# 5l1v3r1/PBS

Hardware: AMD Instinct MI355X
Metric: co-run slowdown (%) vs solo + aggregate throughput, 4-tenant mix at 1/2/4/8 GPU (higher is better)
Workload: dtype bf16

## Files before the change

csrc/hip/runtime.cpp:

```cpp
#include <hip/hip_runtime.h>
#include <hsa/hsa.h>
#include <hsa/hsa_ext_amd.h>
#include <rocprofiler-sdk-roctx/roctx.h>
#include <x86intrin.h>

#include <algorithm>
#include <atomic>
#include <cmath>
#include <cstdio>
#include <cstdlib>
#include <chrono>
#include <condition_variable>
#include <cstring>
#include <deque>
#include <memory>
#include <mutex>
#include <thread>
#include <vector>

#include "../include/gpbs/gpbs.h"
#include "common.hpp"
#include "hwc_attr.h"

using namespace gpbs_hip;

extern "C" {
int gpbs_adapt_update(gpbs_adapt_state_t*, const gpbs_adapt_params_t*, uint64_t, uint64_t, uint64_t, uint64_t);
int gpbs_hip_gemm_units(int, int);
int gpbs_hip_gemm_fp8_units(int, int);
int gpbs_hwc_sample(uint64_t* out, int nxcd);
int gpbs_hwc_sample_se(uint64_t* se_out, uint64_t* x_out);
int gpbs_hwc_slot_per_se(int k);
int gpbs_hwc_active(void);
int gpbs_hip_gemm_bf16(const void*, const void*, void*, int, int, int, void*, const void*, unsigned, unsigned, void*,
                       void*, int, hipStream_t);
int gpbs_hip_gemm_fp8(const void*, const float*, const void*, const float*, void*, int, int, int, int, void*, const void*,
                      unsigned, unsigned, void*, void*, int, hipStream_t);
int gpbs_hip_stream_copy(const void*, void*, unsigned long long, unsigned, void*, const void*, unsigned, unsigned,
                         void*, void*, int, hipStream_t);
int gpbs_hip_reduce_bf16(const void*, const void*, void*, unsigned long long, unsigned, void*, const void*, unsigned,
                         unsigned, void*, void*, int, hipStream_t);
int gpbs_hip_gemv_bf16(const void*, const void*, void*, int, int, void*, const void*, unsigned, unsigned, void*, void*,
                       int, hipStream_t);
int gpbs_hip_partition_switch(void*, unsigned, const unsigned*, hipStream_t);
int gpbs_hip_counter_reduce(void*, void*, const int*, int, void*, hipStream_t);
int gpbs_hip_adapt(void*, const void*, const void*, const void*, int, const gpbs_adapt_params_t*, int*, hipStream_t);
int gpbs_hip_switch_probe(const void*, int, unsigned*, int, unsigned, unsigned long long, hipStream_t);
int gpbs_hip_hwc_attribute(const void*, void*, void*, void*, hipStream_t);
int gpbs_hip_hwc_attribute2(const void*, void*, void*, void*, hipStream_t, int);
int gpbs_hip_allreduce(const void*, unsigned, unsigned long long, unsigned, void*, const void*, unsigned, unsigned,
                       void*, void*, int, unsigned long long, unsigned long long, hipStream_t);
int gpbs_hip_gang_desc_size(void);
int gpbs_hip_gang_exchange(const void*, unsigned, const void*, void*, void*, unsigned long long, hipStream_t);
int gpbs_hip_coll_desc_size(void);
}

namespace {

// ... 110 lines not shown
    return nullptr;
  }
  volatile u32* w = (volatile u32*)p;
  for (int i = 0; i < 1024; ++i) w[i] = 0;
  _mm_sfence();
  return (PartTable*)p;
}

void bar_write(PartTable* b, const u32* owners, u32 epoch);

void bar_sync(PartTable* b, const PartTable* h) {
  *(volatile u32*)&b->flags = __atomic_load_n(&h->flags, __ATOMIC_ACQUIRE);
  *(volatile u32*)&b->hold = __atomic_load_n(&h->hold, __ATOMIC_ACQUIRE);
  bar_write(b, h->owner, __atomic_load_n(&h->epoch, __ATOMIC_ACQUIRE));
}

void bar_write(PartTable* b, const u32* owners, u32 epoch) {
  volatile u32* o = (volatile u32*)b->owner;
  for (int x = 0; x < kXcds * kCtx; ++x) o[x] = owners[x];
  _mm_sfence();
  *(volatile u32*)&b->epoch = epoch;
  _mm_sfence();
}

struct GpuCtx;
void set_hold(GpuCtx* c, u32 v);

struct GpuCtx {
  int device = 0;
  int part_base = 0;
  int table_mode = 0;
  int spatial = 0;
  PartTable* h_table = nullptr;
  PartTable* d_table = nullptr;
  PartTable* b_table = nullptr;
  u64* d_cnt = nullptr;
  bool cnt_bar = false;
  std::atomic<int> cnt_rows{1};
  u64* d_prev = nullptr;
  u64* h_out = nullptr;
  int* h_ids = nullptr;
  gpbs_adapt_state_t* h_states = nullptr;
  u64* h_spin = nullptr;
  int* h_dirs = nullptr;
  u64* h_adelta = nullptr;
  hipStream_t sched_stream = nullptr;
  gpbs_engine_t* engine = nullptr;
  int nctx = 1;
  int waveprio = 0;
  int lat_half = -1;
  int hold_enable = 0;
  std::mutex hold_mu;
  int holds = 0;
  uint64_t hold_gen = 0;
  std::atomic<uint64_t> hold_raises{0};
  std::atomic<int> cls_cache[kMaxTenants];
  u32 pending[kXcds * kCtx];
  u32 epoch = 0;
  bool red_pending = false;
  int red_n = 0;
  int red_buf = 0;
  int* h_ids2 = nullptr;
  u64* h_out2 = nullptr;
  hipEvent_t red_ev = nullptr;
  int hwc = 0;
  int slot_se[kNumPmc] = {1, 1, 1, 0};
  u64* h_blk = nullptr;
  std::vector<u64> snap_blk, blk_prev;
  std::vector<u64> red_prev;
  std::vector<u64> snap_se;
  std::vector<u64> snap_x;
  std::vector<int64_t> snap_own;
  uint64_t snap_seq = 0, used_seq = 0;
  bool hw_primed = false;
// ... 1228 lines not shown
  std::condition_variable cv, idle_cv;
  int64_t pending = 0;
  int64_t inflight = 0;
  bool stop = false;
  std::deque<int64_t> submit_times;
  gpbs_runner_stats_t st{};
  std::vector<int64_t> lats;
  hipEvent_t ev[16];
  int err = 0;
  uint64_t q_hold[16] = {};

  void hold_drop(int qi) {
    if (q_hold[qi]) {
      hold_release(ctx, q_hold[qi] - 1);
      q_hold[qi] = 0;
    }
  }

  std::atomic<int> phase{0};
  uint8_t q_alt[16] = {};
  int cur_alt = 0;
  u32 q_seq[16] = {};
  u32 coll_seq = 0;
  int64_t q_t0[16] = {};

  struct Work {
    int kind, M, N, K, chunk;
    unsigned long long bytes;
    void *a, *b, *c;
  };
  static int coll_timeout_ms(const Work& w) { return w.K > 0 ? w.K : 5000; }
  Work work(int alt) const {
    if (alt && cfg.alt_kind)
      return Work{cfg.alt_kind, cfg.alt_M, cfg.alt_N, cfg.alt_K, cfg.alt_chunk_bytes, cfg.alt_bytes,
                  cfg.alt_a, cfg.alt_b, cfg.alt_c};
    return Work{cfg.kind, cfg.M, cfg.N, cfg.K, cfg.chunk_bytes, cfg.bytes, cfg.a, cfg.b, cfg.c};
  }

  static u32 unit_total(const Work& w) {
    switch (w.kind) {
      case K_ALLREDUCE: {
        const u64 n8 = w.bytes / 16, chunk8 = (u64)w.chunk / 16, per = (n8 + w.M - 1) / w.M;
        const u64 lo = (u64)w.N * per, hi = std::min(lo + per, n8);
        return hi > lo ? (u32)((hi - lo + chunk8 - 1) / chunk8) : 0u;
      }
      case K_GEMM: return (u32)gpbs_hip_gemm_units(w.M, w.N);
      case K_GEMM_FP8: return (u32)gpbs_hip_gemm_fp8_units(w.M, w.N);
      case K_STREAM:
      case K_REDUCE: return (u32)((w.bytes + w.chunk - 1) / w.chunk);
      case K_GEMV: return (u32)((w.M + 15) / 16);
    }
    return 0;
  }

  hipStream_t pick_se_stream() {
    u32 any = 0, bits = 0;
    for (int x = 0; x < kXcds; ++x)
      for (int e = 0; e < kCtx; ++e)
        if ((__atomic_load_n(&ctx->h_table->owner[kCtx * x + e], __ATOMIC_ACQUIRE) & kOwnerMask) == (u32)cfg.tenant) {
          any |= 1u << e;
          bits |= 1u << (kCtx * x + e);
        }
    const int half = (any & ~0x3u) == 0 ? 0 : ((any & ~0xCu) == 0 ? 1 : -1);
    if (!any || half < 0) return stream;
    if (!key_stream || bits != key_bits || half != key_half) {
      uint32_t m[8];
      se_half_mask(half, m);
      if (key_stream) {
        retire_stream(key_stream);
        masked_pool().release(key_stream, key_load);
      }
      const int64_t tnow = mono_ns();
      key_load = rate_t0 && tnow > rate_t0 ? (double)(st.launches - rate_l0) * 1e9 / (double)(tnow - rate_t0) : 0.0;
      rate_t0 = tnow;
      rate_l0 = st.launches;
      key_stream = masked_acquire_key(m, bits, key_load);
// ... 52 lines not shown
    if (!half_stream[k]) half_stream[k] = make_half_stream(k);
    return half_stream[k] ? half_stream[k] : stream;
  }

  int launch(int qi, hipStream_t stream) {
    WorkQueue* q = d_q + qi;
    const Work w = work(q_alt[qi]);
    const int tm = __atomic_load_n(&ctx->table_mode, __ATOMIC_ACQUIRE);
    const bool dev = tm != 0;
    const void* tab = tm == 1 ? (const void*)ctx->d_table : tm == 2 ? (const void*)ctx->b_table : (const void*)ctx->h_table;
    const bool gate = cfg.gate && !ctx->share.load(std::memory_order_acquire);
    const bool hold = gate && ctx->hold_enable && tm != 1 && w.kind != K_GEMV && ctx->engine &&
                      ctx->cls_cache[cfg.tenant].load(std::memory_order_relaxed) == 1;
    const unsigned mode = (gate ? (cfg.gate == 2 ? GATE_PARK : GATE_TABLE) : GATE_NONE) | (dev ? GATE_DEVTABLE : 0) |
                          (gate && ctx->spatial ? GATE_SPATIAL : 0) |
                          (gate && __atomic_load_n(&ctx->se_mode, __ATOMIC_ACQUIRE) ? GATE_SE : 0) |
                          (cfg.priority > 0 && ctx->waveprio ? GATE_WAVEPRIO : 0) | (hold ? GATE_HOLD : 0);
    const unsigned me = (unsigned)cfg.tenant;
    __atomic_store_n(&h_status[qi], 0u, __ATOMIC_RELEASE);
    st.launches++;
    const int grid = cfg.grid ? cfg.grid : cur_grid;
    switch (w.kind) {
      case K_GEMM:
        return gpbs_hip_gemm_bf16(w.a, w.b, w.c, w.M, w.N, w.K, q, tab, mode, me, ctx->d_cnt, &h_status[qi], grid,
                                  stream);
      case K_GEMM_FP8: {
        const char *aq = (const char*)w.a, *bq = (const char*)w.b;
        return gpbs_hip_gemm_fp8(aq, (const float*)(aq + (size_t)w.M * w.K), bq, (const float*)(bq + (size_t)w.N * w.K),
                                 w.c, w.M, w.N, w.K, 0, q, tab, mode, me, ctx->d_cnt, &h_status[qi], grid, stream);
      }
      case K_STREAM:
        return gpbs_hip_stream_copy(w.a, w.c, w.bytes, (unsigned)w.chunk, q, tab, mode, me, ctx->d_cnt,
                                    &h_status[qi], grid, stream);
      case K_REDUCE:
        return gpbs_hip_reduce_bf16(w.a, w.b, w.c, w.bytes, (unsigned)w.chunk, q, tab, mode, me, ctx->d_cnt,
                                    &h_status[qi], grid, stream);
      case K_GEMV:
        return gpbs_hip_gemv_bf16(w.a, w.b, w.c, w.M, w.K, q, tab, mode, me, ctx->d_cnt, &h_status[qi], grid,
                                  stream);
      case K_ALLREDUCE:
        return gpbs_hip_allreduce(w.a, q_seq[qi], w.bytes, (unsigned)w.chunk, q, tab, mode, me, ctx->d_cnt,
                                  &h_status[qi], grid, (unsigned long long)coll_timeout_ms(w) * 100000ull,
                                  100000ull, stream);
    }
    return -22;
  }

  bool owns_any() {
    if (!cfg.gate || shared()) return true;
    for (int x = 0; x < kXcds * kCtx; ++x)
      if ((__atomic_load_n(&ctx->h_table->owner[x], __ATOMIC_ACQUIRE) & kOwnerMask) == (u32)cfg.tenant) return true;
    return false;
  }

  int wo_qi = -1;
  int64_t q_l0[16] = {};
  int64_t drain_seen_rv = 0;
  int64_t ramp_from = 0;
  static void ewma(std::atomic<int64_t>& a, std::atomic<uint64_t>& n, int64_t v) {
    const int64_t o = a.load(std::memory_order_relaxed);
    a.store(n.load(std::memory_order_relaxed) ? o + (v - o) / 8 : v, std::memory_order_relaxed);
    n.fetch_add(1, std::memory_order_relaxed);
  }
  void note_drain(int qi, int64_t now) {
    if (cfg.tenant < 0 || cfg.tenant >= kMaxTenants) return;
    const int64_t rv = ctx->revoke_ns[cfg.tenant].load(std::memory_order_relaxed);
    if (!rv || rv == drain_seen_rv || rv < q_l0[qi] || now < rv) return;
    const u32 s = __atomic_load_n(&h_status[qi], __ATOMIC_ACQUIRE);
    if ((s & 0x80000000u) && (s & 0x3fffffffu) >= unit_total(work(q_alt[qi]))) return;
    drain_seen_rv = rv;
    const int64_t dr = now - rv;
    if (dr >= 1000000000) return;
    st.drain_sum_ns += dr;
    st.drain_count++;
    if (dr > st.drain_max_ns) st.drain_max_ns = dr;
    ewma(ctx->swc_drain_ns[cfg.tenant], ctx->swc_drain_n[cfg.tenant], dr);
  }
  void note_ramp(int64_t now) {
    if (!ramp_from || cfg.tenant < 0 || cfg.tenant >= kMaxTenants) return;
    const int64_t g = ctx->grant_ns[cfg.tenant].load(std::memory_order_relaxed);
    if (g >= ramp_from && now >= g && now - g < 1000000000)
      ewma(ctx->swc_ramp_ns[cfg.tenant], ctx->swc_ramp_n[cfg.tenant], now - g);
    ramp_from = 0;
  }

  void wait_owner() {
    if (owns_any()) return;
    st.waits_owner++;
    const int64_t t0 = mono_ns();
    ramp_from = t0;
    int watch = wo_qi;
    std::unique_lock<std::mutex> lk(ctx->mu);
// ... 49 lines not shown
            std::lock_guard<std::mutex> g(mu);
            if (pending <= 0) break;
            for (int k = 0; k < nq; ++k) {
              int cand = (next_q + k) % nq;
              if (!q_busy[cand]) {
                qi = cand;
                break;
              }
            }
            if (qi < 0) break;
            fresh = true;
          }
          wo_qi = fl.empty() ? -1 : fl.front().qi;
          wait_owner();
          if (stop) break;
          if (fresh) {
            q_alt[qi] = (uint8_t)(cfg.alt_kind && phase.load(std::memory_order_acquire));
            q_seq[qi] = coll_seq++;
            q_t0[qi] = mono_ns();
          }
          cur_alt = q_alt[qi];
          hipStream_t stream = pick_stream();
          if (fresh) {
            std::lock_guard<std::mutex> g(mu);
            pending--;
            inflight++;
            next_q = (qi + 1) % nq;
            q_busy[qi] = 1;
          } else {
            relaunch.pop_front();
            st.relaunches++;
          }
          if (cfg.priority > 0 && ctx->hold_enable && fresh && !q_hold[qi]) q_hold[qi] = hold_acquire(ctx) + 1;
          q_l0[qi] = mono_ns();
          note_ramp(q_l0[qi]);
          if (launch(qi, stream) != 0) err = -5;
          const int e = qi;
          hipEventRecord(ev[e], stream);
          fl.push_back({qi, e});
        }
        if (fl.empty()) {
          std::lock_guard<std::mutex> g(mu);
          if (pending <= 0 && relaunch.empty()) break;
          continue;
        }
        Fl f = fl.front();
        fl.pop_front();
        while (hipEventQuery(ev[f.ev]) == hipErrorNotReady) {
          if (stop) break;
          std::this_thread::yield();
        }
        const u32 s = __atomic_load_n(&h_status[f.qi], __ATOMIC_ACQUIRE);
        const u32 done = s & 0x3fffffffu;
        const Work fw = work(q_alt[f.qi]);
        const bool unfinished = !((s & 0x80000000u) && done >= unit_total(fw));
        const bool coll_late = fw.kind == K_ALLREDUCE && unfinished &&
                               mono_ns() - q_t0[f.qi] > (int64_t)coll_timeout_ms(fw) * 1000000;
        if (((s & 0x80000000u) && (s & 0x40000000u)) || coll_late) {
          std::fprintf(stderr, "[gpbs-hip] tenant %d: collective unit %u timed out waiting for its peers\n",
                       cfg.tenant, q_seq[f.qi]);
          err = -110;
          hold_drop(f.qi);
          std::lock_guard<std::mutex> g(mu);
          q_busy[f.qi] = 0;
          inflight--;
          pending = 0;
          if (!submit_times.empty()) submit_times.pop_front();
        } else if ((s & 0x80000000u) && done >= unit_total(work(q_alt[f.qi]))) {
          hold_drop(f.qi);
          const int64_t t = mono_ns();
          std::lock_guard<std::mutex> g(mu);
          q_busy[f.qi] = 0;
          inflight--;
          st.units_done++;
          st.units_alt += q_alt[f.qi];
          st.last_done_ns = t;
          if (!submit_times.empty()) {
            const int64_t lat = t - submit_times.front();
            submit_times.pop_front();
            st.lat_sum_ns += lat;
            st.lat_count++;
            if (lat > st.lat_max_ns) st.lat_max_ns = lat;
            if (lats.size() < (1u << 20)) lats.push_back(lat);
          }
        } else {
          relaunch.push_back(f.qi);
          note_drain(f.qi, mono_ns());
        }
        if (stop) break;
      }
      st.busy_ns += mono_ns() - batch_t0;
      {
        std::lock_guard<std::mutex> g(mu);
        if (pending <= 0 && inflight <= 0) {
          engine_wake(false);
          idle_cv.notify_all();
        }
      }
      if (stop) break;
    }
// ... 758 lines not shown
  hipFree(d_st);
  return rc;
}

int gpbs_gpu_param(void* p, const char* name, int value) {
  GpuCtx* c = (GpuCtx*)p;
  if (!c || !name) return -22;
  struct Ent {
    const char* n;
    int* f;
    int lo, hi;
  };
  const Ent tab[] = {
      {"period_us", &c->hwc_period_us, 100, 1000000},   {"slow_us", &c->hwc_slow_us, 0, 10000000},
      {"duty_pct", &c->hwc_duty_pct, 0, 100},           {"burst_ms", &c->hwc_burst_ms, 0, 10000},
      {"budget_pct", &c->hwc_budget_pct, 0, 100},       {"bucket", &c->hwc_bucket, 1, 100000},
      {"clean_pct", &c->clean_pct, 0, 100},             {"device_attr", &c->dev_attr, 0, 1},
      {"fallback", &c->model_fallback, 0, 1},           {"stale_us", &c->hwc_stale_us, 0, 100000000},
      {"watch", &c->hwc_watch, 0, 1},                   {"align", &c->hwc_align, 0, 1},
      {"guard_us", &c->hwc_guard_us, 0, 100000},        {"long_us", &c->hwc_long_us, 0, 100000000},
      {"pair_gap_us", &c->hwc_pair_gap_us, 0, 10000000}, {"measure_ms", &c->hwc_measure_ms, 0, 100000},
      {"share", &c->share_enable, 0, 1},                {"probe_every", &c->probe_every, 0, 1000000},
      {"probe_len", &c->probe_len, 0, 1000000},         {"cadence", &c->model_cadence, 0, 1},
  };
  for (const Ent& e : tab)
    if (std::strcmp(e.n, name) == 0) {
      std::lock_guard<std::mutex> g(c->snap_mu);
      const int old = *e.f;
      if (value >= 0) {
        if (e.f == &c->dev_attr && (value != 0) != (old != 0)) {
          if (c->attr_pending) {
            hipEventSynchronize(c->attr_ev);
            hwc_fold(c, *c->h_aout, c->mod_inflight, c->pres_inflight, c->t_inflight);
            c->attr_pending = false;
          }
          c->hw_primed = false;
        }
        *e.f = std::max(e.lo, std::min(e.hi, value));
        if (e.f == &c->hwc_bucket || e.f == &c->hwc_budget_pct) c->hwc_tokens = c->hwc_bucket;
      }
      return old;
    }
  return -22;
}

int gpbs_gpu_hwc_reset(void* p) {
// ... 987 lines not shown
```

csrc/hip/tenant_kernels.hip:

```cpp
#include "common.hpp"

namespace gpbs_hip {


__device__ __forceinline__ int grab_unit_x(WorkQueue* q, const PartTable* table, u32 mode, u32 me, u32 xcc,
                                           int* s_slot, u32 total) {
  if (threadIdx.x == 0) {
    int u = -1;
    hold_wait(table, mode);
    const u32 per = (total + kXcds - 1) / kXcds;
    for (u32 spins = 0;; ++spins) {
      if (owns(table, mode, me, xcc)) {
        for (u32 k = 0; k < (u32)kXcds; ++k) {
          const u32 r = (xcc + k) & (kXcds - 1);
          const u32 lo = r * per, hi = min(lo + per, total);
          if (lo >= hi) continue;
          if (__hip_atomic_load(&q->xnext[r], __ATOMIC_RELAXED, __HIP_MEMORY_SCOPE_AGENT) >= hi - lo) continue;
          const u32 t = atomicAdd(&q->xnext[r], 1u);
          if (t < hi - lo) {
            u = (int)(lo + t);
            atomicAdd(&q->next, 1u);
            break;
          }
        }
// ... 12 lines not shown
  __syncthreads();
  int u = *s_slot;
  __syncthreads();
  return u;
}


__device__ __forceinline__ u16 f2bf(float x) { return __builtin_bit_cast(u16, (__bf16)x); }
__device__ __forceinline__ float bf2f(u16 x) { return __uint_as_float(((u32)x) << 16); }

constexpr int GBM = 128, GBN = 128, GBK = 64, GNT = 256;
constexpr int kGemmLds = 2 * 2 * GBM * GBK * 2;

typedef __attribute__((address_space(3))) char lds_t;

__device__ __forceinline__ void glds16(const void* g, lds_t* l) {
  __builtin_amdgcn_global_load_lds(g, (__attribute__((address_space(3))) void*)l, 16, 0, 0);
}

__global__ __launch_bounds__(GNT, 2) void k_gemm_bf16_tn(const u16* __restrict__ A, const u16* __restrict__ Bt,
                                                         u16* __restrict__ C, int M, int N, int K, WorkQueue* q,
                                                         const PartTable* table, u32 mode, u32 me, u64* cnt,
                                                         u32 inst_per_tile, u32 refs_per_tile, u32 miss_per_tile,
                                                         u32* status) {
  __shared__ __attribute__((aligned(16))) char smem[kGemmLds + 16];
  lds_t* lds = (lds_t*)smem;
  int* s_slot = (int*)(smem + kGemmLds);
  const u32 xcc = xcc_id();
  u64 t_last = __builtin_amdgcn_s_memtime();
  const int tid = threadIdx.x, lane = tid & 63, wid = tid >> 6;
  const int wr = wid >> 1, wc = wid & 1;
  const int tiles_m = M / GBM, tiles_n = N / GBN, ntiles = tiles_m * tiles_n;
  const int nk = K / GBK;
  constexpr int GROUP_M = 8;

  int srow[4], scol[4];
#pragma unroll
  for (int j = 0; j < 4; ++j) {
    const int c = wid * 4 + j;
    srow[j] = 8 * c + (lane >> 3);
    scol[j] = (((lane & 7) ^ (srow[j] & 7)) * 8);
  }

  for (;;) {
    const int t = grab_unit(q, table, mode, me, xcc, s_slot, (u32)ntiles);
    if (t < 0) break;
    const int in_group = GROUP_M * tiles_n;
    const int g = t / in_group;
    const int first_m = g * GROUP_M;
    const int gsz = min(tiles_m - first_m, GROUP_M);
    const int tm = first_m + (t % in_group) % gsz;
    const int tn = (t % in_group) / gsz;
    const u16* Ab = A + (size_t)tm * GBM * K;
    const u16* Bb = Bt + (size_t)tn * GBN * K;

    f32x4 acc[4][4];
#pragma unroll
    for (int i = 0; i < 4; ++i)
#pragma unroll
      for (int j = 0; j < 4; ++j) acc[i][j] = f32x4{0.f, 0.f, 0.f, 0.f};

    auto stage = [&](int buf, int kt) {
      lds_t* la = lds + buf * (2 * GBM * GBK * 2);
      lds_t* lb = la + GBM * GBK * 2;
#pragma unroll
      for (int j = 0; j < 4; ++j) {
        const int c = wid * 4 + j;
        glds16(Ab + (size_t)srow[j] * K + kt * GBK + scol[j], la + c * 1024);
        glds16(Bb + (size_t)srow[j] * K + kt * GBK + scol[j], lb + c * 1024);
// ... 19 lines not shown
          const int rb = wc * 64 + i * 16 + (lane & 15);
          b[i] = *(const __attribute__((address_space(3))) bf16x8*)(lb + rb * 128 + ((chunk ^ (rb & 7)) << 4));
        }
#pragma unroll
        for (int i = 0; i < 4; ++i)
#pragma unroll
          for (int j = 0; j < 4; ++j) acc[i][j] = __builtin_amdgcn_mfma_f32_16x16x32_bf16(a[i], b[j], acc[i][j], 0, 0, 0);
      }
      asm volatile("s_waitcnt vmcnt(0)" ::: "memory");
      __syncthreads();
      cur ^= 1;
    }
#pragma unroll
    for (int i = 0; i < 4; ++i)
#pragma unroll
      for (int j = 0; j < 4; ++j) {
        const int m = tm * GBM + wr * 64 + i * 16 + (lane >> 4) * 4;
        const int n = tn * GBN + wc * 64 + j * 16 + (lane & 15);
#pragma unroll
        for (int r = 0; r < 4; ++r) C[(size_t)(m + r) * N + n] = f2bf(acc[i][j][r]);
      }
    count_unit(cnt, me, xcc, inst_per_tile, &t_last, refs_per_tile, miss_per_tile, q);
  }
  finish(q, status, (u32)ntiles);
}

constexpr int G2_BM = 256, G2_BK = 64, G2_NT = 512;
constexpr u32 kGemmXRange = 1u << 16;
constexpr u32 kGemmBlock2D = 1u << 17;
constexpr u32 kGemmStatic = 1u << 18;
constexpr int kGemmOptsLive = 1 | 8 | 1 << 23;
constexpr int kGemmOptsShipped = 256 | 8192 | 65536 | 131072;
static int g_gemm_opts = 8;
constexpr int kG2Half = 128 * 128;
constexpr int kG2Buf = 4 * kG2Half;
constexpr int kG2Lds = 2 * kG2Buf;

__device__ __forceinline__ int g2_swz(int r) { return (r >> 1) & 7; }

__global__ __launch_bounds__(G2_NT, 1) void k_gemm256_bf16_tn(const u16* __restrict__ A, const u16* __restrict__ Bt,
                                                             u16* __restrict__ C, int M, int N, int K, WorkQueue* q,
                                                             const PartTable* table, u32 mode, u32 me, u64* cnt,
                                                             u32 inst_per_tile, u32 refs_per_tile, u32 miss_per_tile,
                                                             u32* status) {
  __shared__ __attribute__((aligned(16))) char smem[kG2Lds + 16];
  lds_t* lds = (lds_t*)smem;
  int* s_slot = (int*)(smem + kG2Lds);
  const u32 xcc = xcc_id();
  u64 t_last = __builtin_amdgcn_s_memtime();
  const int tid = threadIdx.x, lane = tid & 63, wid = tid >> 6;
  const int wu = __builtin_amdgcn_readfirstlane(wid);
  const int wr = wu >> 2, wc = wu & 3;
  const int tiles_m = M / G2_BM, tiles_n = N / G2_BM, ntiles = tiles_m * tiles_n;
  const int nt = K / G2_BK;
  int soff[2];
#pragma unroll
  for (int j = 0; j < 2; ++j) {
    const int row = 8 * (2 * wid + j) + (lane >> 3);
    soff[j] = row * K + (((lane & 7) ^ g2_swz(row)) * 8);
  }
  int soffa[4];
#pragma unroll
  for (int j = 0; j < 4; ++j) {
    const int row = 8 * (4 * (wid & 3) + j) + (lane >> 3);
    soffa[j] = row * K + (((lane & 7) ^ g2_swz(row)) * 8);
  }
  const int l16 = lane & 15, lq = lane >> 4;
  const int bh = wc >> 1, bc = (wc & 1) * 64;
  int units_seen = 0;

  for (;;) {
    const int tile = (mode & kGemmStatic) ? (units_seen ? -1 : (int)blockIdx.x)
                     : (mode & kGemmXRange) ? grab_unit_x(q, table, mode, me, xcc, s_slot, (u32)ntiles)
                                            : grab_unit(q, table, mode, me, xcc, s_slot, (u32)ntiles);
    if (tile < 0) break;
    int tm = tile / tiles_n, tn = tile % tiles_n;
    if ((mode & kGemmBlock2D) && (tiles_m & 3) == 0 && (tiles_n & 1) == 0 && ntiles % kXcds == 0) {
      const int per = ntiles / kXcds;
      const int bm = tiles_m / 4, bn = tiles_n / 2;
      const int g = (mode & kGemmXRange) ? tile / per : tile % kXcds;
      const int jj = (mode & kGemmXRange) ? tile % per : tile / kXcds;
      tm = (g >> 1) * bm + jj / bn;
      tn = (g & 1) * bn + jj % bn;
    }
    const u16* Ab = A + (size_t)tm * G2_BM * K;
    const u16* Bb = Bt + (size_t)tn * G2_BM * K;
    auto stage = [&](int kind, int h, int t) {
      const u16* src = (kind ? Bb : Ab) + (size_t)h * 128 * K + t * G2_BK;
      lds_t* dst = lds + (t & 1) * kG2Buf + (kind * 2 + h) * kG2Half + wid * 2048;
      glds16(src + soff[0], dst);
      glds16(src + soff[1], dst + 1024);
    };
    auto stage_own_a = [&](int t) {
      const u16* src = Ab + (size_t)wr * 128 * K + t * G2_BK;
      lds_t* dst = lds + (t & 1) * kG2Buf + wr * kG2Half + (wid & 3) * 4096;
#pragma unroll
      for (int j = 0; j < 4; ++j) glds16(src + soffa[j], dst + j * 1024);
    };
    auto frag = [&](int b, int kind, int h, int r0, int s) -> bf16x8 {
      const int r = r0 + l16;
      const lds_t* p = lds + b * kG2Buf + (kind * 2 + h) * kG2Half + r * 128 + (((4 * s + lq) ^ g2_swz(r)) << 4);
      return *(const __attribute__((address_space(3))) bf16x8*)p;
    };
    f32x4 acc[8][4];
#pragma unroll
    for (int i = 0; i < 8; ++i)
#pragma unroll
      for (int j = 0; j < 4; ++j) acc[i][j] = f32x4{0.f, 0.f, 0.f, 0.f};
    stage(1, 0, 0); stage(1, 1, 0); stage(0, 0, 0); stage(0, 1, 0);
    asm volatile("s_waitcnt vmcnt(0)" ::: "memory");
    __builtin_amdgcn_s_barrier();
    if (wr == 1) __builtin_amdgcn_s_barrier();
    bf16x8 a[4][2], b[4][2];
    for (int t = 0; t < nt; ++t) {
      const int buf = t & 1;
      const bool more = t + 1 < nt;
#pragma unroll
      for (int j = 0; j < 4; ++j)
#pragma unroll
        for (int s2 = 0; s2 < 2; ++s2) b[j][s2] = frag(buf, 1, bh, bc + j * 16, s2);
      __builtin_amdgcn_sched_barrier(0);
#pragma unroll
      for (int i = 0; i < 4; ++i)
#pragma unroll
        for (int s2 = 0; s2 < 2; ++s2) a[i][s2] = frag(buf, 0, wr, i * 16, s2);
      if (more) {
        stage(1, 0, t + 1); stage(1, 1, t + 1);
      } else {
        asm volatile("s_waitcnt vmcnt(0)" ::: "memory");
      }
      __builtin_amdgcn_s_barrier();
      asm volatile("s_waitcnt lgkmcnt(0)" ::: "memory");
      __builtin_amdgcn_s_setprio(1);
#pragma unroll
      for (int s2 = 0; s2 < 2; ++s2)
#pragma unroll
        for (int i = 0; i < 4; ++i)
#pragma unroll
          for (int j = 0; j < 4; ++j)
            acc[i][j] = __builtin_amdgcn_mfma_f32_16x16x32_bf16(b[j][s2], a[i][s2], acc[i][j], 0, 0, 0);
      __builtin_amdgcn_s_setprio(0);
      __builtin_amdgcn_s_barrier();
#pragma unroll
      for (int i = 0; i < 4; ++i)
#pragma unroll
        for (int s2 = 0; s2 < 2; ++s2) a[i][s2] = frag(buf, 0, wr, 64 + i * 16, s2);
      if (more) {
        stage_own_a(t + 1);
        asm volatile("s_waitcnt vmcnt(4)" ::: "memory");
      }
      __builtin_amdgcn_s_barrier();
      asm volatile("s_waitcnt lgkmcnt(0)" ::: "memory");
      __builtin_amdgcn_s_setprio(1);
#pragma unroll
      for (int s2 = 0; s2 < 2; ++s2)
#pragma unroll
        for (int i = 0; i < 4; ++i)
#pragma unroll
          for (int j = 0; j < 4; ++j)
            acc[4 + i][j] = __builtin_amdgcn_mfma_f32_16x16x32_bf16(b[j][s2], a[i][s2], acc[4 + i][j], 0, 0, 0);
      __builtin_amdgcn_s_setprio(0);
      asm volatile("s_waitcnt vmcnt(0)" ::: "memory");
      __builtin_amdgcn_s_barrier();
    }
    if (wr == 0) __builtin_amdgcn_s_barrier();
#pragma unroll
    for (int i = 0; i < 8; ++i)
#pragma unroll
      for (int j = 0; j < 4; ++j) {
        const int m = wr * 128 + i * 16 + l16;
        const int c8 = wc * 16 + j * 4 + lq;
        const u32 lo = (u32)f2bf(acc[i][j][0]) | ((u32)f2bf(acc[i][j][1]) << 16);
        const u32 hi = (u32)f2bf(acc[i][j][2]) | ((u32)f2bf(acc[i][j][3]) << 16);
        *(__attribute__((address_space(3))) u32x2*)(lds + m * 512 + ((c8 ^ (m & 15)) << 3)) = u32x2{lo, hi};
      }
    __syncthreads();
#pragma unroll
    for (int p = 0; p < 16; ++p) {
      const int row = p * 16 + (tid >> 5), c16 = tid & 31;
      u32x4 v = *(const __attribute__((address_space(3))) u32x4*)(lds + row * 512 + (((2 * c16) ^ (row & 14)) << 3));
      if (row & 1) v = u32x4{v.z, v.w, v.x, v.y};
      u32x4* dst = (u32x4*)(C + (size_t)(tm * G2_BM + row) * N + tn * G2_BM + c16 * 8);
      __builtin_nontemporal_store(v, dst);
    }
    __syncthreads();
    ++units_seen;
    if (!(mode & kGemmStatic)) count_unit(cnt, me, xcc, inst_per_tile, &t_last, refs_per_tile, miss_per_tile, q);
  }
  if (!(mode & kGemmStatic)) finish(q, status, (u32)ntiles);
}

constexpr int SNT = 256, SUNROLL = 16, RUNROLL = 6;

template <int U, bool NTS>
__global__ __launch_bounds__(SNT) void k_stream_copy(const f32x4* __restrict__ src, f32x4* __restrict__ dst,
                                                    u64 n4, u32 chunk4, WorkQueue* q, const PartTable* table, u32 mode,
                                                    u32 me, u64* cnt, u32* status) {
  __shared__ int s_slot[4];
  const u32 xcc = xcc_id();
  u64 t_last = __builtin_amdgcn_s_memtime();
  const u32 nchunks = (u32)((n4 + chunk4 - 1) / chunk4);
  const u64 lines = (u64)chunk4 * 16 / 128;
  const u64 inst = (u64)chunk4 * 2 / 64 + 8;
  for (;;) {
    const int c = grab_unit(q, table, mode, me, xcc, s_slot, nchunks);
    if (c < 0) break;
    const u64 base = (u64)c * chunk4;
    const u64 end = min(base + chunk4, n4);
    for (u64 i = base + threadIdx.x; i < end; i += (u64)SNT * U) {
      f32x4 v[U];
#pragma unroll
      for (int k = 0; k < U; ++k) {
// ... 159 lines not shown
extern "C" {

int gpbs_hip_set_gemm_opts(int opts) {
  const int old = g_gemm_opts;
  if (opts < 0) return old;
  const int gone = opts & ~(kGemmOptsLive | kGemmOptsShipped);
  static bool warned = false;
  if (gone && !warned) {
    warned = true;
    fprintf(stderr,
            "gpbs_hip_set_gemm_opts: bits 0x%x select GEMM variants that were removed (docs/gemm_lab.md); "
            "the shipped schedule runs\n",
            gone);
  }
  g_gemm_opts = opts & kGemmOptsLive;
  return old;
}

int gpbs_hip_gemm_units(int M, int N) {
  if (M % G2_BM == 0 && N % G2_BM == 0) return (M / G2_BM) * (N / G2_BM);
  return (M / GBM) * (N / GBN);
}

int gpbs_hip_gemm_bf16(const void* A, const void* Bt, void* C, int M, int N, int K, void* q, const void* table,
                       unsigned mode, unsigned me, void* cnt, void* status, int grid, hipStream_t s) {
  if (M % GBM || N % GBN || K % GBK || M <= 0 || N <= 0 || K <= 0) return -22;
  if (M % G2_BM == 0 && N % G2_BM == 0) {
    const int ntiles = (M / G2_BM) * (N / G2_BM);
    if (grid <= 0) grid = 256;
    if (grid > ntiles) grid = ntiles;
    const u32 inst = (u32)((G2_BM / 16) * (G2_BM / 16) * (K / 32) + (K / G2_BK) * 64 + 128);
    const u32 refs = (u32)(((u64)2 * G2_BM * K * 2) / 128);
    const u32 miss = (u32)((((u64)M + N) * K * 2 / 128) / ntiles + (u64)G2_BM * G2_BM * 2 / 128);
    const u32 m2 = mode | ((g_gemm_opts & 1) ? kGemmXRange : 0u) |
                   ((g_gemm_opts & 8) && ntiles % kXcds == 0 ? kGemmBlock2D : 0u) |
                   ((g_gemm_opts & (1 << 23)) && (mode & 3) == GATE_NONE && grid == ntiles ? kGemmStatic : 0u);
    hipLaunchKernelGGL(k_gemm256_bf16_tn, dim3(grid), dim3(G2_NT), 0, s, (const u16*)A, (const u16*)Bt, (u16*)C, M, N,
                       K, (WorkQueue*)q, (const PartTable*)table, m2, me, (u64*)cnt, inst, refs, miss, (u32*)status);
    return hipGetLastError() == hipSuccess ? 0 : -5;
  }
  const int ntiles = (M / GBM) * (N / GBN);
  if (grid <= 0) grid = 256 * 2;
  if (grid > ntiles) grid = ntiles;
  const u32 inst = (u32)((GBM / 16) * (GBN / 16) * (K / 32) * 2 + (K / GBK) * 32 + 64);
  const u32 refs = (u32)(((u64)(GBM + GBN) * K * 2) / 128);
  const u32 miss = (u32)((((u64)M + N) * K * 2 / 128) / ntiles + (u64)GBM * GBN * 2 / 128);
  hipLaunchKernelGGL(k_gemm_bf16_tn, dim3(grid), dim3(GNT), 0, s, (const u16*)A, (const u16*)Bt, (u16*)C, M, N, K,
                     (WorkQueue*)q, (const PartTable*)table, mode, me, (u64*)cnt, inst, refs, miss, (u32*)status);
  return hipGetLastError() == hipSuccess ? 0 : -5;
}

static int g_stream_opts = 0;

int gpbs_hip_set_stream_opts(int opts) {
  const int old = g_stream_opts;
  if (opts >= 0) g_stream_opts = opts;
  return old;
}

int gpbs_hip_stream_copy(const void* src, void* dst, unsigned long long bytes, unsigned chunk_bytes, void* q,
                         const void* table, unsigned mode, unsigned me, void* cnt, void* status, int grid, hipStream_t s) {
  if (bytes % 16 || chunk_bytes % 16 || chunk_bytes == 0) return -22;
  if (grid <= 0) grid = 256;
  using K = void (*)(const f32x4*, f32x4*, u64, u32, WorkQueue*, const PartTable*, u32, u32, u64*, u32*);
  static const K tab[4] = {k_stream_copy<SUNROLL, true>, k_stream_copy<SUNROLL, false>, k_stream_copy<8, true>,
                           k_stream_copy<8, false>};
  hipLaunchKernelGGL(tab[g_stream_opts & 3], dim3(grid), dim3(SNT), 0, s, (const f32x4*)src, (f32x4*)dst, bytes / 16,
                     chunk_bytes / 16, (WorkQueue*)q, (const PartTable*)table, mode, me, (u64*)cnt, (u32*)status);
  return hipGetLastError() == hipSuccess ? 0 : -5;
}

static int g_reduce_opts = 8;
// ... 42 lines not shown
```

pbs_amd/core/config.py:

```python
from __future__ import annotations

import os
from typing import Any, Dict

try:
    import tomllib as _toml
except ImportError:
    import tomli as _toml

REFERENCE_PROFILE: Dict[str, Any] = dict(
    sched="credit", tslice_us=100, ratelimit_us=1000, metric_period_us=1000,
    adapt=dict(threshold=100, band_lo=70, band_hi=130, min_us=100, max_us=1100, inc_us=100, dec_us=200,
               switch_boundary=900, ticks_per_tslice=3),
)

MI355X_PROFILE: Dict[str, Any] = dict(
    sched="credit", tslice_us=1000, ratelimit_us=250, metric_period_us=1000, quantum_align_us=250,
    coschedule=3, class_period_us=2000,
    class_pin_us=2000000,
    region_q=0, region_vt=1, switch_floor_x=200, switch_floor_max_us=30000, shared_q_us=0, slo_cap=0,
    probe_max_us=50000,
    mem_split=2,
    adapt=dict(threshold=20000, band_lo=70, band_hi=130, min_us=1000, max_us=11000, inc_us=1000, dec_us=2000,
               switch_boundary=9000, ticks_per_tslice=3,
               grow_pct=0),
    atc=dict(wait_unit_ns=8),
)

RUNTIME_KEYS = ("period_us", "slow_us", "duty_pct", "burst_ms", "budget_pct", "bucket", "clean_pct", "device_attr",
                "fallback", "stale_us", "watch", "align", "guard_us", "long_us", "pair_gap_us", "measure_ms", "share",
                "probe_every", "probe_len")

BOOT_KEYS = ("sched", "tslice_us", "ratelimit_us", "smt_power_savings", "tickle_one_idle", "default_yield",
             "migration_delay_us", "metric_period_us", "slice_apply_us", "pmu_refresh_us", "dom0_quirk",
             "heartbeat_timeout_us", "trace_capacity", "quantum_align_us", "coschedule", "class_period_us",
             "boost_exclusive", "class_split", "idle_skip", "class_dwell", "class_budget", "present_us",
             "sibling_steal", "class_steal", "class_fall", "shared_q_us", "class_pin_us", "region_q", "switch_floor_x",
             "switch_floor_max_us", "region_vt", "slo_cap", "probe_max_us", "mem_split")


def load(path: str | None = None, profile: Dict[str, Any] | None = None) -> Dict[str, Any]:
    base = dict(profile or REFERENCE_PROFILE)
    cfg: Dict[str, Any] = {"boot": {k: v for k, v in base.items() if k not in ("adapt", "atc")},
                           "policy": dict(base.get("adapt", {})), "atc": dict(base.get("atc", {})),
                           "tenants": {}, "pools": {}, "runtime": {}}
    if path:
        with open(path, "rb") as f:
            doc = _toml.load(f)
        cfg["boot"].update(doc.get("boot", {}))
        cfg["policy"].update(doc.get("policy", {}))
        cfg["atc"].update(doc.get("atc", {}))
        cfg["tenants"].update(doc.get("tenant", {}))
        cfg["pools"].update(doc.get("pool", {}))
        rt = doc.get("runtime", {})
# ... 15 lines not shown
```

pbs_amd/ops/hipabi.py:

```python
from __future__ import annotations

import ctypes as C

from .. import _native as N

u32, i32, u64, i64 = C.c_uint32, C.c_int32, C.c_uint64, C.c_int64
vp = C.c_void_p


class RunnerCfg(C.Structure):
    _fields_ = [(n, C.c_int) for n in ("kind", "tenant", "gate", "priority", "depth", "grid", "M", "N", "K",
                                       "chunk_bytes", "engine_wake", "reserved")] + \
               [("bytes", C.c_ulonglong), ("a", vp), ("b", vp), ("c", vp)] + \
               [(n, C.c_int) for n in ("alt_kind", "alt_M", "alt_N", "alt_K", "alt_chunk_bytes", "alt_reserved")] + \
               [("alt_bytes", C.c_ulonglong), ("alt_a", vp), ("alt_b", vp), ("alt_c", vp)]


class RunnerStats(C.Structure):
    _fields_ = [(n, u64) for n in ("units_done", "launches", "relaunches", "waits_owner", "submitted")] + \
               [(n, i64) for n in ("busy_ns", "wait_owner_ns", "first_start_ns", "last_done_ns", "lat_sum_ns",
                                   "lat_max_ns")] + [("lat_count", u64), ("units_alt", u64)] + \
               [("drain_sum_ns", i64), ("drain_max_ns", i64), ("drain_count", u64)]


KIND = {"gemm": 1, "stream": 2, "reduce": 3, "gemv": 4, "allreduce": 5, "gemm_fp8": 6}


def _p(lib, name, res, *args):
    f = getattr(lib, name)
    f.restype = res
    f.argtypes = list(args)


def bind(lib):
    _p(lib, "gpbs_roctx_push", C.c_int, C.c_char_p)
    _p(lib, "gpbs_roctx_pop", C.c_int)
    _p(lib, "gpbs_roctx_mark", None, C.c_char_p)
    _p(lib, "gpbs_gpu_switch_latency", C.c_int, vp, C.c_int, C.c_int, vp)
    _p(lib, "gpbs_hip_gemm_bf16", C.c_int, vp, vp, vp, C.c_int, C.c_int, C.c_int, vp, vp, C.c_uint, C.c_uint, vp, vp,
       C.c_int, vp)
    _p(lib, "gpbs_hip_gemm_fp8", C.c_int, vp, vp, vp, vp, vp, C.c_int, C.c_int, C.c_int, C.c_int, vp, vp, C.c_uint,
       C.c_uint, vp, vp, C.c_int, vp)
    _p(lib, "gpbs_hip_gemm_fp8_units", C.c_int, C.c_int, C.c_int)
    _p(lib, "gpbs_hip_stream_copy", C.c_int, vp, vp, C.c_ulonglong, C.c_uint, vp, vp, C.c_uint, C.c_uint, vp, vp,
       C.c_int, vp)
    _p(lib, "gpbs_hip_reduce_bf16", C.c_int, vp, vp, vp, C.c_ulonglong, C.c_uint, vp, vp, C.c_uint, C.c_uint, vp, vp,
       C.c_int, vp)
    _p(lib, "gpbs_hip_gemv_bf16", C.c_int, vp, vp, vp, C.c_int, C.c_int, vp, vp, C.c_uint, C.c_uint, vp, vp, C.c_int,
       vp)
    _p(lib, "gpbs_hip_set_gemm_opts", C.c_int, C.c_int)
    _p(lib, "gpbs_hip_set_reduce_opts", C.c_int, C.c_int)
    _p(lib, "gpbs_hip_set_stream_opts", C.c_int, C.c_int)
    _p(lib, "gpbs_hwc_init", C.c_int, C.c_char_p)
    _p(lib, "gpbs_hwc_init_gpu", C.c_int, C.c_char_p, C.c_int)
    _p(lib, "gpbs_hwc_start", C.c_int)
    _p(lib, "gpbs_hwc_active", C.c_int)
    _p(lib, "gpbs_hwc_trace_enable", C.c_int, C.c_int)
    _p(lib, "gpbs_hwc_trace_stats", C.c_int, C.c_char_p, C.c_int, C.c_int)
    _p(lib, "gpbs_hwc_sample", C.c_int, C.POINTER(C.c_uint64), C.c_int)
    _p(lib, "gpbs_hwc_stop", C.c_int)
    _p(lib, "gpbs_gpu_set_hwc", C.c_int, vp, C.c_int)
    _p(lib, "gpbs_gpu_hwc_stats", C.c_int, vp, C.POINTER(C.c_uint64), C.POINTER(C.c_uint64), C.POINTER(C.c_double))
    _p(lib, "gpbs_hwc_sample_se", C.c_int, C.POINTER(C.c_uint64), C.POINTER(C.c_uint64))
# ... 111 lines not shown
```

Before: 1.258.

## Batch multiple GEMM work units per launch and prefetch next tile ticket

The runner can now hand several pending GEMM requests to a single persistent-kernel launch, sized by a new gemm_batch knob (default 8). It does this only when the tenant is not time-shared and does not cover the latency lane. The kernel treats tile tickets modulo the tile count, so one launch covers units × tiles, which amortises per-launch and status-polling overhead. The 256-tile kernel also grabs the next ticket during the last K step, hiding the queue atomic latency. In exchange, latency accounting is coarser because a whole batch completes together, and preemption and drain granularity grow with batch size.

```diff
diff --git a/csrc/hip/runtime.cpp b/csrc/hip/runtime.cpp
--- a/csrc/hip/runtime.cpp
+++ b/csrc/hip/runtime.cpp
@@ -34,6 +34,9 @@
 int gpbs_hwc_active(void);
 int gpbs_hip_gemm_bf16(const void*, const void*, void*, int, int, int, void*, const void*, unsigned, unsigned, void*,
                        void*, int, hipStream_t);
+int gpbs_hip_gemm_bf16_batch(const void*, const void*, void*, int, int, int, int, void*, const void*, unsigned, unsigned,
+                             void*, void*, int, hipStream_t);
+int gpbs_hip_gemm_batch_units(int);
 int gpbs_hip_gemm_fp8(const void*, const float*, const void*, const float*, void*, int, int, int, int, void*, const void*,
                       unsigned, unsigned, void*, void*, int, hipStream_t);
 int gpbs_hip_stream_copy(const void*, void*, unsigned long long, unsigned, void*, const void*, unsigned, unsigned,
@@ -190,6 +193,8 @@
   *(volatile u32*)&b->epoch = epoch;
   _mm_sfence();
 }
+
+constexpr int kGemmBatchDefault = 8;
 
 struct GpuCtx;
 void set_hold(GpuCtx* c, u32 v);
@@ -218,6 +223,7 @@
   int waveprio = 0;
   int lat_half = -1;
   int hold_enable = 0;
+  int gemm_batch = kGemmBatchDefault;
   std::mutex hold_mu;
   int holds = 0;
   uint64_t hold_gen = 0;
@@ -1492,6 +1498,7 @@
   int cur_alt = 0;
   u32 q_seq[16] = {};
   u32 coll_seq = 0;
+  u32 q_units[16] = {};
   int64_t q_t0[16] = {};
 
   struct Work {
@@ -1522,6 +1529,7 @@
     }
     return 0;
   }
+  u32 slot_total(int qi) const { return unit_total(work(q_alt[qi])) * (q_units[qi] ? q_units[qi] : 1u); }
 
   hipStream_t pick_se_stream() {
     u32 any = 0, bits = 0;
@@ -1620,8 +1628,8 @@
     const int grid = cfg.grid ? cfg.grid : cur_grid;
     switch (w.kind) {
       case K_GEMM:
-        return gpbs_hip_gemm_bf16(w.a, w.b, w.c, w.M, w.N, w.K, q, tab, mode, me, ctx->d_cnt, &h_status[qi], grid,
-                                  stream);
+        return gpbs_hip_gemm_bf16_batch(w.a, w.b, w.c, w.M, w.N, w.K, (int)q_units[qi], q, tab, mode, me, ctx->d_cnt,
+                                        &h_status[qi], grid, stream);
       case K_GEMM_FP8: {
         const char *aq = (const char*)w.a, *bq = (const char*)w.b;
         return gpbs_hip_gemm_fp8(aq, (const float*)(aq + (size_t)w.M * w.K), bq, (const float*)(bq + (size_t)w.N * w.K),
@@ -1665,7 +1673,7 @@
     const int64_t rv = ctx->revoke_ns[cfg.tenant].load(std::memory_order_relaxed);
     if (!rv || rv == drain_seen_rv || rv < q_l0[qi] || now < rv) return;
     const u32 s = __atomic_load_n(&h_status[qi], __ATOMIC_ACQUIRE);
-    if ((s & 0x80000000u) && (s & 0x3fffffffu) >= unit_total(work(q_alt[qi]))) return;
+    if ((s & 0x80000000u) && (s & 0x3fffffffu) >= slot_total(qi)) return;
     drain_seen_rv = rv;
     const int64_t dr = now - rv;
     if (dr >= 1000000000) return;
@@ -1761,9 +1769,18 @@
           cur_alt = q_alt[qi];
           hipStream_t stream = pick_stream();
           if (fresh) {
+            const int lh = __atomic_load_n(&ctx->lat_half, __ATOMIC_ACQUIRE);
+            const bool confined = key_stream && stream == key_stream;
+            const bool covers_lane = lh >= 0 && !(confined && key_half != (lh & 1));
+            const bool time_shared = cfg.gate && !shared() && !confined;
+            const int64_t want = work(cur_alt).kind == K_GEMM && !covers_lane && !time_shared
+                                     ? gpbs_hip_gemm_batch_units(__atomic_load_n(&ctx->gemm_batch, __ATOMIC_RELAXED))
+                                     : 1;
             std::lock_guard<std::mutex> g(mu);
-            pending--;
-            inflight++;
+            const int64_t n = std::min<int64_t>(want, std::max<int64_t>(pending, 1));
+            q_units[qi] = (u32)n;
+            pending -= n;
+            inflight += n;
             next_q = (qi + 1) % nq;
             q_busy[qi] = 1;
           } else {
@@ -1792,7 +1809,7 @@
         const u32 s = __atomic_load_n(&h_status[f.qi], __ATOMIC_ACQUIRE);
         const u32 done = s & 0x3fffffffu;
         const Work fw = work(q_alt[f.qi]);
-        const bool unfinished = !((s & 0x80000000u) && done >= unit_total(fw));
+        const bool unfinished = !((s & 0x80000000u) && done >= slot_total(f.qi));
         const bool coll_late = fw.kind == K_ALLREDUCE && unfinished &&
                                mono_ns() - q_t0[f.qi] > (int64_t)coll_timeout_ms(fw) * 1000000;
         if (((s & 0x80000000u) && (s & 0x40000000u)) || coll_late) {
@@ -1802,19 +1819,20 @@
           hold_drop(f.qi);
           std::lock_guard<std::mutex> g(mu);
           q_busy[f.qi] = 0;
-          inflight--;
+          inflight -= q_units[f.qi];
           pending = 0;
-          if (!submit_times.empty()) submit_times.pop_front();
-        } else if ((s & 0x80000000u) && done >= unit_total(work(q_alt[f.qi]))) {
+          for (u32 k = 0; k < q_units[f.qi] && !submit_times.empty(); ++k) submit_times.pop_front();
+        } else if (!unfinished) {
           hold_drop(f.qi);
           const int64_t t = mono_ns();
           std::lock_guard<std::mutex> g(mu);
           q_busy[f.qi] = 0;
-          inflight--;
-          st.units_done++;
-          st.units_alt += q_alt[f.qi];
+          const u32 n = q_units[f.qi];
+          inflight -= n;
+          st.units_done += n;
+          st.units_alt += (uint64_t)q_alt[f.qi] * n;
           st.last_done_ns = t;
-          if (!submit_times.empty()) {
+          for (u32 k = 0; k < n && !submit_times.empty(); ++k) {
             const int64_t lat = t - submit_times.front();
             submit_times.pop_front();
             st.lat_sum_ns += lat;
@@ -2619,6 +2637,7 @@
       {"pair_gap_us", &c->hwc_pair_gap_us, 0, 10000000}, {"measure_ms", &c->hwc_measure_ms, 0, 100000},
       {"share", &c->share_enable, 0, 1},                {"probe_every", &c->probe_every, 0, 1000000},
       {"probe_len", &c->probe_len, 0, 1000000},         {"cadence", &c->model_cadence, 0, 1},
+      {"gemm_batch", &c->gemm_batch, 1, 64},
   };
   for (const Ent& e : tab)
     if (std::strcmp(e.n, name) == 0) {
diff --git a/csrc/hip/tenant_kernels.hip b/csrc/hip/tenant_kernels.hip
--- a/csrc/hip/tenant_kernels.hip
+++ b/csrc/hip/tenant_kernels.hip
@@ -58,7 +58,7 @@
                                                          u16* __restrict__ C, int M, int N, int K, WorkQueue* q,
                                                          const PartTable* table, u32 mode, u32 me, u64* cnt,
                                                          u32 inst_per_tile, u32 refs_per_tile, u32 miss_per_tile,
-                                                         u32* status) {
+                                                         u32* status, u32 units) {
   __shared__ __attribute__((aligned(16))) char smem[kGemmLds + 16];
   lds_t* lds = (lds_t*)smem;
   int* s_slot = (int*)(smem + kGemmLds);
@@ -68,6 +68,7 @@
   const int wr = wid >> 1, wc = wid & 1;
   const int tiles_m = M / GBM, tiles_n = N / GBN, ntiles = tiles_m * tiles_n;
   const int nk = K / GBK;
+  const u32 total = units * (u32)ntiles;
   constexpr int GROUP_M = 8;
 
   int srow[4], scol[4];
@@ -79,8 +80,9 @@
   }
 
   for (;;) {
-    const int t = grab_unit(q, table, mode, me, xcc, s_slot, (u32)ntiles);
-    if (t < 0) break;
+    const int ticket = grab_unit(q, table, mode, me, xcc, s_slot, total);
+    if (ticket < 0) break;
+    const int t = ticket % ntiles;
     const int in_group = GROUP_M * tiles_n;
     const int g = t / in_group;
     const int first_m = g * GROUP_M;
@@ -146,14 +148,16 @@
       }
     count_unit(cnt, me, xcc, inst_per_tile, &t_last, refs_per_tile, miss_per_tile, q);
   }
-  finish(q, status, (u32)ntiles);
+  finish(q, status, total);
 }
 
 constexpr int G2_BM = 256, G2_BK = 64, G2_NT = 512;
 constexpr u32 kGemmXRange = 1u << 16;
 constexpr u32 kGemmBlock2D = 1u << 17;
 constexpr u32 kGemmStatic = 1u << 18;
-constexpr int kGemmOptsLive = 1 | 8 | 1 << 23;
+constexpr u32 kGemmNoPrefetch = 1u << 19;
+constexpr int kNoTicket = -2;
+constexpr int kGemmOptsLive = 1 | 8 | 1 << 23 | 1 << 24;
 constexpr int kGemmOptsShipped = 256 | 8192 | 65536 | 131072;
 static int g_gemm_opts = 8;
 constexpr int kG2Half = 128 * 128;
@@ -166,7 +170,7 @@
                                                              u16* __restrict__ C, int M, int N, int K, WorkQueue* q,
                                                              const PartTable* table, u32 mode, u32 me, u64* cnt,
                                                              u32 inst_per_tile, u32 refs_per_tile, u32 miss_per_tile,
-                                                             u32* status) {
+                                                             u32* status, u32 units) {
   __shared__ __attribute__((aligned(16))) char smem[kG2Lds + 16];
   lds_t* lds = (lds_t*)smem;
   int* s_slot = (int*)(smem + kG2Lds);
@@ -177,6 +181,7 @@
   const int wr = wu >> 2, wc = wu & 3;
   const int tiles_m = M / G2_BM, tiles_n = N / G2_BM, ntiles = tiles_m * tiles_n;
   const int nt = K / G2_BK;
+  const u32 total = units * (u32)ntiles;
   int soff[2];
 #pragma unroll
   for (int j = 0; j < 2; ++j) {
@@ -192,12 +197,16 @@
   const int l16 = lane & 15, lq = lane >> 4;
   const int bh = wc >> 1, bc = (wc & 1) * 64;
   int units_seen = 0;
+  int ahead = kNoTicket;
+  const bool prefetch = !(mode & (kGemmStatic | kGemmXRange | kGemmNoPrefetch | GATE_HOLD));
 
   for (;;) {
-    const int tile = (mode & kGemmStatic) ? (units_seen ? -1 : (int)blockIdx.x)
-                     : (mode & kGemmXRange) ? grab_unit_x(q, table, mode, me, xcc, s_slot, (u32)ntiles)
-                                            : grab_unit(q, table, mode, me, xcc, s_slot, (u32)ntiles);
-    if (tile < 0) break;
+    const int ticket = ahead != kNoTicket          ? ahead
+                       : (mode & kGemmStatic)      ? (units_seen ? -1 : (int)blockIdx.x)
+                       : (mode & kGemmXRange)      ? grab_unit_x(q, table, mode, me, xcc, s_slot, total)
+                                                   : grab_unit(q, table, mode, me, xcc, s_slot, total);
+    if (ticket < 0) break;
+    const int tile = ticket % ntiles;
     int tm = tile / tiles_n, tn = tile % tiles_n;
     if ((mode & kGemmBlock2D) && (tiles_m & 3) == 0 && (tiles_n & 1) == 0 && ntiles % kXcds == 0) {
       const int per = ntiles / kXcds;
@@ -239,6 +248,8 @@
     for (int t = 0; t < nt; ++t) {
       const int buf = t & 1;
       const bool more = t + 1 < nt;
+      u32 pre = 0;
+      bool pre_taken = false;
 #pragma unroll
       for (int j = 0; j < 4; ++j)
 #pragma unroll
@@ -252,6 +263,10 @@
         stage(1, 0, t + 1); stage(1, 1, t + 1);
       } else {
         asm volatile("s_waitcnt vmcnt(0)" ::: "memory");
+        if (prefetch && wu == 0 && lane == 0 && owns(table, mode, me, xcc)) {
+          pre = atomicInc(&q->next, 0xFFFFFFFFu);
+          pre_taken = true;
+        }
       }
       __builtin_amdgcn_s_barrier();
       asm volatile("s_waitcnt lgkmcnt(0)" ::: "memory");
@@ -285,6 +300,7 @@
             acc[4 + i][j] = __builtin_amdgcn_mfma_f32_16x16x32_bf16(b[j][s2], a[i][s2], acc[4 + i][j], 0, 0, 0);
       __builtin_amdgcn_s_setprio(0);
       asm volatile("s_waitcnt vmcnt(0)" ::: "memory");
+      if (!more && wu == 0 && lane == 0) *s_slot = pre_taken ? (pre < total ? (int)pre : -1) : kNoTicket;
       __builtin_amdgcn_s_barrier();
     }
     if (wr == 0) __builtin_amdgcn_s_barrier();
@@ -299,6 +315,7 @@
         *(__attribute__((address_space(3))) u32x2*)(lds + m * 512 + ((c8 ^ (m & 15)) << 3)) = u32x2{lo, hi};
       }
     __syncthreads();
+    ahead = *s_slot;
 #pragma unroll
     for (int p = 0; p < 16; ++p) {
       const int row = p * 16 + (tid >> 5), c16 = tid & 31;
@@ -311,7 +328,7 @@
     ++units_seen;
     if (!(mode & kGemmStatic)) count_unit(cnt, me, xcc, inst_per_tile, &t_last, refs_per_tile, miss_per_tile, q);
   }
-  if (!(mode & kGemmStatic)) finish(q, status, (u32)ntiles);
+  if (!(mode & kGemmStatic)) finish(q, status, total);
 }
 
 constexpr int SNT = 256, SUNROLL = 16, RUNROLL = 6;
@@ -517,9 +534,13 @@
   return (M / GBM) * (N / GBN);
 }
 
-int gpbs_hip_gemm_bf16(const void* A, const void* Bt, void* C, int M, int N, int K, void* q, const void* table,
-                       unsigned mode, unsigned me, void* cnt, void* status, int grid, hipStream_t s) {
-  if (M % GBM || N % GBN || K % GBK || M <= 0 || N <= 0 || K <= 0) return -22;
+int gpbs_hip_gemm_batch_units(int want) { return (g_gemm_opts & 1) || want < 1 ? 1 : want; }
+
+int gpbs_hip_gemm_bf16_batch(const void* A, const void* Bt, void* C, int M, int N, int K, int units, void* q,
+                             const void* table, unsigned mode, unsigned me, void* cnt, void* status, int grid,
+                             hipStream_t s) {
+  if (M % GBM || N % GBN || K % GBK || M <= 0 || N <= 0 || K <= 0 || units < 1 || units > 4096) return -22;
+  units = gpbs_hip_gemm_batch_units(units);
   if (M % G2_BM == 0 && N % G2_BM == 0) {
     const int ntiles = (M / G2_BM) * (N / G2_BM);
     if (grid <= 0) grid = 256;
@@ -527,11 +548,14 @@
     const u32 inst = (u32)((G2_BM / 16) * (G2_BM / 16) * (K / 32) + (K / G2_BK) * 64 + 128);
     const u32 refs = (u32)(((u64)2 * G2_BM * K * 2) / 128);
     const u32 miss = (u32)((((u64)M + N) * K * 2 / 128) / ntiles + (u64)G2_BM * G2_BM * 2 / 128);
-    const u32 m2 = mode | ((g_gemm_opts & 1) ? kGemmXRange : 0u) |
+    const u32 m2 = mode | ((g_gemm_opts & 1) ? kGemmXRange : 0u) | ((g_gemm_opts & (1 << 24)) ? kGemmNoPrefetch : 0u) |
                    ((g_gemm_opts & 8) && ntiles % kXcds == 0 ? kGemmBlock2D : 0u) |
-                   ((g_gemm_opts & (1 << 23)) && (mode & 3) == GATE_NONE && grid == ntiles ? kGemmStatic : 0u);
+                   ((g_gemm_opts & (1 << 23)) && (mode & 3) == GATE_NONE && grid == ntiles && units == 1 && !status
+                        ? kGemmStatic
+                        : 0u);
     hipLaunchKernelGGL(k_gemm256_bf16_tn, dim3(grid), dim3(G2_NT), 0, s, (const u16*)A, (const u16*)Bt, (u16*)C, M, N,
-                       K, (WorkQueue*)q, (const PartTable*)table, m2, me, (u64*)cnt, inst, refs, miss, (u32*)status);
+                       K, (WorkQueue*)q, (const PartTable*)table, m2, me, (u64*)cnt, inst, refs, miss, (u32*)status,
+                       (u32)units);
     return hipGetLastError() == hipSuccess ? 0 : -5;
   }
   const int ntiles = (M / GBM) * (N / GBN);
@@ -541,8 +565,14 @@
   const u32 refs = (u32)(((u64)(GBM + GBN) * K * 2) / 128);
   const u32 miss = (u32)((((u64)M + N) * K * 2 / 128) / ntiles + (u64)GBM * GBN * 2 / 128);
   hipLaunchKernelGGL(k_gemm_bf16_tn, dim3(grid), dim3(GNT), 0, s, (const u16*)A, (const u16*)Bt, (u16*)C, M, N, K,
-                     (WorkQueue*)q, (const PartTable*)table, mode, me, (u64*)cnt, inst, refs, miss, (u32*)status);
+                     (WorkQueue*)q, (const PartTable*)table, mode, me, (u64*)cnt, inst, refs, miss, (u32*)status,
+                     (u32)units);
   return hipGetLastError() == hipSuccess ? 0 : -5;
+}
+
+int gpbs_hip_gemm_bf16(const void* A, const void* Bt, void* C, int M, int N, int K, void* q, const void* table,
+                       unsigned mode, unsigned me, void* cnt, void* status, int grid, hipStream_t s) {
+  return gpbs_hip_gemm_bf16_batch(A, Bt, C, M, N, K, 1, q, table, mode, me, cnt, status, grid, s);
 }
 
 static int g_stream_opts = 0;
diff --git a/pbs_amd/core/config.py b/pbs_amd/core/config.py
--- a/pbs_amd/core/config.py
+++ b/pbs_amd/core/config.py
@@ -29,7 +29,7 @@
 
 RUNTIME_KEYS = ("period_us", "slow_us", "duty_pct", "burst_ms", "budget_pct", "bucket", "clean_pct", "device_attr",
                 "fallback", "stale_us", "watch", "align", "guard_us", "long_us", "pair_gap_us", "measure_ms", "share",
-                "probe_every", "probe_len")
+                "probe_every", "probe_len", "gemm_batch")
 
 BOOT_KEYS = ("sched", "tslice_us", "ratelimit_us", "smt_power_savings", "tickle_one_idle", "default_yield",
              "migration_delay_us", "metric_period_us", "slice_apply_us", "pmu_refresh_us", "dom0_quirk",
diff --git a/pbs_amd/ops/hipabi.py b/pbs_amd/ops/hipabi.py
--- a/pbs_amd/ops/hipabi.py
+++ b/pbs_amd/ops/hipabi.py
@@ -39,6 +39,9 @@
     _p(lib, "gpbs_gpu_switch_latency", C.c_int, vp, C.c_int, C.c_int, vp)
     _p(lib, "gpbs_hip_gemm_bf16", C.c_int, vp, vp, vp, C.c_int, C.c_int, C.c_int, vp, vp, C.c_uint, C.c_uint, vp, vp,
        C.c_int, vp)
+    _p(lib, "gpbs_hip_gemm_bf16_batch", C.c_int, vp, vp, vp, C.c_int, C.c_int, C.c_int, C.c_int, vp, vp, C.c_uint,
+       C.c_uint, vp, vp, C.c_int, vp)
+    _p(lib, "gpbs_hip_gemm_batch_units", C.c_int, C.c_int)
     _p(lib, "gpbs_hip_gemm_fp8", C.c_int, vp, vp, vp, vp, vp, C.c_int, C.c_int, C.c_int, C.c_int, vp, vp, C.c_uint,
        C.c_uint, vp, vp, C.c_int, vp)
     _p(lib, "gpbs_hip_gemm_fp8_units", C.c_int, C.c_int, C.c_int)
```

Result: no change. 1.259 (median of 2 runs) (+0.0%).
